# jurihock/sdft

Measured on AMD Instinct MI355X. Metric: Msamples/s analysis+synthesis, m=1024 Hann fp64; achieved HBM GB/s vs peak, higher is better.
Workload: dtype f64

## Files before the change

### sdft_amd/csrc/sdft_forward.hpp

```cpp

#pragma once

#include "sdft_carry_exact.hpp"

#pragma clang fp contract(off)

namespace sdfthip {

template <typename FD, int WIN> SDFT_D cx<FD> window_tap(cx<FD> m2, cx<FD> m1, cx<FD> c0, cx<FD> p1, cx<FD> p2, FD w)
{
  if constexpr (WIN == WIN_HANN)
  {
    const cx<FD> a = cadd(c0, c0);
    const cx<FD> b = cadd(m1, p1);
    return cscale(csub(a, b), w);
  }
  else if constexpr (WIN == WIN_HAMMING)
  {
    const cx<FD> a = cscale(c0, (FD)(0.54));
    const cx<FD> b = cscale(cadd(m1, p1), (FD)(0.23));
    return cscale(csub(a, b), w);
  }
  else if constexpr (WIN == WIN_BLACKMAN)
  {
    const cx<FD> a = cscale(c0, (FD)(0.42));
    const cx<FD> b = cscale(cadd(m1, p1), (FD)(0.25));
    const cx<FD> d = cscale(cadd(m2, p2), (FD)(0.04));
    return cscale(cadd(csub(a, b), d), w);
  }
  else
  {
    return cscale(c0, w);
  }
}

template <typename FD, int WIN> SDFT_D cx<FD> window_tap_fused(cx<FD> m2, cx<FD> m1, cx<FD> c0, cx<FD> p1, cx<FD> p2, FD w)
{
  if constexpr (WIN == WIN_HANN)
  {
    const cx<FD> b = cadd(m1, p1);
    const FD w2 = w + w;
    return cmake<FD>(__builtin_fma(c0.re, w2, -(b.re * w)), __builtin_fma(c0.im, w2, -(b.im * w)));
  }
  else if constexpr (WIN == WIN_HAMMING)
  {
    const cx<FD> b = cadd(m1, p1);
    const FD wa = (FD)(0.54) * w, wb = (FD)(0.23) * w;
    return cmake<FD>(__builtin_fma(c0.re, wa, -(b.re * wb)), __builtin_fma(c0.im, wa, -(b.im * wb)));
  }
  else if constexpr (WIN == WIN_BLACKMAN)
  {
    const cx<FD> b = cadd(m1, p1);
    const cx<FD> d = cadd(m2, p2);
    const FD wa = (FD)(0.42) * w, wb = (FD)(0.25) * w, wd = (FD)(0.04) * w;
    return cmake<FD>(__builtin_fma(d.re, wd, __builtin_fma(c0.re, wa, -(b.re * wb))),
                     __builtin_fma(d.im, wd, __builtin_fma(c0.im, wa, -(b.im * wb))));
  }
  else
  {
    return cscale(c0, w);
  }
}

template <typename FD> SDFT_D cx<FD> fid_from_table(const cx<FD>* fseed, unsigned L, unsigned nbins, long kk, unsigned c, cx<FD> tw)
{
  cx<FD> f = fseed[(size_t)(c / L) * nbins + kk];
  for (unsigned i = c % L; i > 0; --i) f = cmul(f, tw);
  return f;
}

template <typename FD> struct ForwardArgs
{
  const FD* delta;
  const cx<FD>* tw;
  const cx<FD>* wtab;
  const cx<FD>* carry;
  const cx<FD>* seed;
  const cx<FD>* fseed;
  unsigned fseed_L;
  cx<FD>* out;
  size_t out_stride;
  cx<FD>* const* out_rows;
  cx<FD>* acc_state;
  cx<FD>* fid_state;
  size_t n;
  unsigned long long total_waves;
  unsigned nbins, chunks, chunk_len, tiles, interior_lanes, cursor0;
  unsigned chunk0, launch_chunks;
  unsigned chunk_shift;
  int vec_store;
  FD wscale;
  DoneSignal done;
  const unsigned* ready;
  unsigned ready_seq, ready_n, ready_channels;
  unsigned* ready_status;
  unsigned ready_status_seen;
  unsigned xcd_map;
  unsigned inv_chunks, inv_channels;
};
SDFT_D unsigned xcd_contiguous(unsigned b, unsigned total)
{
  const unsigned q = total >> 3, r = total & 7u, x = b & 7u;
  return x * q + (x < r ? x : r) + (b >> 3);
}

SDFT_D void uniform_divmod(unsigned block, unsigned d, unsigned inv, unsigned& q, unsigned& r)
{
  if (inv == 0) { q = block; r = 0; return; }
  q = __builtin_amdgcn_readfirstlane((unsigned)(((unsigned long long)block * inv) >> 32));
  r = block - q * d;
  if (r >= d) { --q; r += d; }
}
template <typename FD> SDFT_D void flow_position(const ForwardArgs<FD>& a, unsigned& chunk, size_t& ch, unsigned block)
{
  unsigned q, r;
  if (a.ready) { uniform_divmod(block, a.ready_channels, a.inv_channels, q, r); chunk = a.chunk0 + q; ch = r; }
  else
  {
    if (a.xcd_map) block = xcd_contiguous(block, a.xcd_map);
    uniform_divmod(block, a.launch_chunks, a.inv_chunks, q, r);
    chunk = a.chunk0 + r; ch = q;
  }
}
template <typename FD> SDFT_D void flow_position(const ForwardArgs<FD>& a, unsigned& chunk, size_t& ch) { flow_position(a, chunk, ch, blockIdx.x); }
constexpr unsigned kFlowPollCap = 1u << 19;
template <typename FD> SDFT_D bool flow_wait(const ForwardArgs<FD>& a, unsigned chunk, size_t ch)
{
  if (!a.ready) return true;
  const unsigned* row = a.ready + (ch * a.chunks + chunk) * (size_t)a.ready_n;
  for (unsigned polls = 0;; ++polls)
  {
    bool ok = true;
    for (unsigned i = threadIdx.x; i < a.ready_n; i += blockDim.x)
      ok = ok && __hip_atomic_load(row + i, __ATOMIC_RELAXED, __HIP_MEMORY_SCOPE_AGENT) == a.ready_seq;
    if (__syncthreads_and(ok ? 1 : 0)) break;
    if (polls > kFlowPollCap)
    {
      if (threadIdx.x == 0 && a.ready_status) __hip_atomic_fetch_add(a.ready_status, 1u, __ATOMIC_RELAXED, __HIP_MEMORY_SCOPE_SYSTEM);
      return false;
    }
    if ((polls & 1023u) == 1023u && a.ready_status)
    {
      const bool gone = threadIdx.x == 0 && __hip_atomic_load(a.ready_status, __ATOMIC_RELAXED, __HIP_MEMORY_SCOPE_SYSTEM) != a.ready_status_seen;
      if (__syncthreads_or(gone ? 1 : 0)) return false;
    }
    __builtin_amdgcn_s_sleep(32);
  }
  __builtin_amdgcn_fence(__ATOMIC_ACQUIRE, "agent");
  asm volatile("s_waitcnt vmcnt(0)" ::: "memory");
  __syncthreads();
  return true;
}

template <typename TD, typename FD> struct SelfArgs
{
  const TD* x;
  size_t x_stride;
  const TD* hist_in;
  TD* hist_out;
  const cx<FD>* acc_in;
  unsigned log2m;
  unsigned lds_deltas;
  const FD* prefix;
#ifdef SDFT_SELF_STAMPS
  unsigned long long* stamps;
#endif
  RadixList rl;
};

template <int CP, int QB, typename TD, typename FD>
SDFT_D void self_fold(const SelfArgs<TD, FD>& sa, cx<FD>* cells, unsigned m, unsigned cursor0, size_t ch, size_t t0)
{
  const TD* xs = sa.x + ch * sa.x_stride;
  const TD* hs = sa.hist_in + ch * (size_t)m;
  const unsigned nthr = blockDim.x;
  const size_t rows = (t0 + m - 1) / m;
  for (unsigned v0 = threadIdx.x; v0 < m; v0 += CP * nthr)
  {
    size_t tv[CP]; FD sum[CP]; TD prev[CP];
#pragma unroll
    for (int c = 0; c < CP; ++c)
    {
      const unsigned v = v0 + (unsigned)c * nthr;
      tv[c] = (size_t)(((v < m ? v : v0) + m - cursor0) % m);
      sum[c] = (FD)0;
      prev[c] = hs[tv[c]];
    }
    for (size_t q = 0; q < rows; q += QB)
    {
      TD cur[CP][QB];
#pragma unroll
      for (int c = 0; c < CP; ++c)
#pragma unroll
        for (int qq = 0; qq < QB; ++qq)
        {
          const size_t t = tv[c] + (q + qq) * (size_t)m;
          cur[c][qq] = xs[t < t0 ? t : t0 - 1];
        }
#pragma unroll
      for (int c = 0; c < CP; ++c)
#pragma unroll
        for (int qq = 0; qq < QB; ++qq)
        {
          const size_t t = tv[c] + (q + qq) * (size_t)m;
          if (t < t0) { const TD dd = cur[c][qq] - prev[c]; sum[c] += (FD)dd; prev[c] = cur[c][qq]; }
        }
    }
#pragma unroll
    for (int c = 0; c < CP; ++c)
    {
      const unsigned v = v0 + (unsigned)c * nthr;
      if (v < m) cells[v] = cmake<FD>(sum[c], (FD)0);
    }
  }
}

template <typename FD>
SDFT_D void lds_fft_dif(cx<FD>* x, unsigned log2m, const cx<FD>* __restrict__ w)
{
  const unsigned m = 1u << log2m;
  unsigned st = 0;
  for (; st + 2 <= log2m; st += 2)
  {
    const unsigned half = m >> (st + 1), quarter = half >> 1;
    for (unsigned i = threadIdx.x; i < (m >> 2); i += blockDim.x)
    {
      const unsigned pos = i & (quarter - 1);
      const unsigned base = ((i - pos) << 2) + pos;
      const cx<FD> a0 = x[base], a1 = x[base + quarter], a2 = x[base + half], a3 = x[base + half + quarter];
      const cx<FD> w1 = w[(size_t)pos << st];
      const cx<FD> w2 = w[(size_t)pos << (st + 1)];
      const cx<FD> b0 = cadd(a0, a2), b2 = cmul(csub(a0, a2), w1);
      const cx<FD> b1 = cadd(a1, a3), tq = cmul(csub(a1, a3), w1);
      const cx<FD> b3 = cmake<FD>(tq.im, -tq.re);
      x[base] = cadd(b0, b1);
      x[base + quarter] = cmul(csub(b0, b1), w2);
      x[base + half] = cadd(b2, b3);
      x[base + half + quarter] = cmul(csub(b2, b3), w2);
    }
    __syncthreads();
  }
  if (st < log2m)
  {
    for (unsigned i = threadIdx.x; i < (m >> 1); i += blockDim.x)
    {
      const cx<FD> p = x[2 * i], q = x[2 * i + 1];
      x[2 * i] = cadd(p, q);
      x[2 * i + 1] = csub(p, q);
    }
    __syncthreads();
  }
}

template <typename FD>
SDFT_D cx<FD>* lds_fft_mixed(cx<FD>* x, unsigned m, const RadixList& rl, const cx<FD>* __restrict__ w)
{
  cx<FD>* y = x + m;
  unsigned ns = 1;
  for (unsigned st = 0; st < rl.count; ++st)
  {
    const unsigned r = rl.r[st];
    const unsigned nr = m / r;
    const unsigned tstep = m / (ns * r);
    const unsigned rstep = nr;
    for (unsigned i = threadIdx.x; i < nr; i += blockDim.x)
    {
      const unsigned k = i % ns;
      cx<FD> v[5];
#pragma unroll
      for (unsigned t = 0; t < 5; ++t)
        if (t < r)
        {
          const cx<FD> in = x[i + t * nr];
          v[t] = t == 0 ? in : cmul(in, w[(size_t)(((unsigned long long)t * k * tstep) % m)]);
        }
      const unsigned base = (i / ns) * ns * r + k;
#pragma unroll
      for (unsigned q = 0; q < 5; ++q)
        if (q < r)
        {
          cx<FD> o = v[0];
#pragma unroll
          for (unsigned t = 1; t < 5; ++t)
            if (t < r) o = cadd(o, cmul(v[t], w[(size_t)(((unsigned long long)q * t * rstep) % m)]));
          y[base + q * ns] = o;
        }
    }
    __syncthreads();
    cx<FD>* tmp = x; x = y; y = tmp;
    ns *= r;
  }
  return x;
}

template <typename TD, typename FD> SDFT_D unsigned self_slot(const SelfArgs<TD, FD>& sa, unsigned k)
{
  return sa.log2m ? (__brev(k) >> (32u - sa.log2m)) : k;
}
template <int CP, int QB, typename TD, typename FD>
SDFT_D cx<FD>* self_carry(const SelfArgs<TD, FD>& sa, const ForwardArgs<FD>& a, cx<FD>* cells, unsigned chunk, size_t ch, size_t t0)
{
  const unsigned m = 2u * a.nbins;
  if (chunk + 1 == a.chunks && sa.hist_out)
  {
    const TD* xv = sa.x + ch * sa.x_stride;
    const TD* hv = sa.hist_in + ch * (size_t)m;
    TD* ho = sa.hist_out + ch * (size_t)m;
    for (size_t i = threadIdx.x; i < m; i += blockDim.x)
    {
      const size_t q = a.n + i;
      ho[i] = (q >= m) ? xv[q - m] : hv[q];
    }
  }
  if (t0 == 0) return nullptr;
#ifdef SDFT_SELF_STAMPS
  const bool st_on = sa.stamps && chunk + 1 == a.chunks && threadIdx.x == 0;
  if (st_on) sa.stamps[1] = __builtin_readcyclecounter();
#endif
  if (sa.prefix)
  {
    const FD* pc = sa.prefix + (ch * a.chunks + chunk) * (size_t)m;
    for (unsigned v = threadIdx.x; v < m; v += blockDim.x) cells[v] = cmake<FD>(pc[v], (FD)0);
  }
  else self_fold<CP, QB>(sa, cells, m, a.cursor0, ch, t0);
  __syncthreads();
#ifdef SDFT_SELF_STAMPS
  if (st_on) sa.stamps[2] = __builtin_readcyclecounter();
#endif
  if (sa.log2m)
  {
    lds_fft_dif(cells, sa.log2m, a.wtab);
#ifdef SDFT_SELF_STAMPS
    if (st_on) sa.stamps[3] = __builtin_readcyclecounter();
#endif
    return cells;
  }
  return lds_fft_mixed(cells, m, sa.rl, a.wtab);
}

template <int G, typename TD, typename FD>
SDFT_D void self_deltas(FD (&dl)[G], const SDFT_CONSTANT TD* xs, const SDFT_CONSTANT TD* hs, size_t tt, size_t span)
{
  TD cur[G], old[G];
#pragma unroll
  for (int u = 0; u < G; ++u) cur[u] = xs[tt + u];
  if (tt + G <= span)
  {
#pragma unroll
    for (int u = 0; u < G; ++u) old[u] = hs[tt + u];
  }
  else if (tt >= span)
  {
#pragma unroll
    for (int u = 0; u < G; ++u) old[u] = xs[tt - span + u];
  }
  else
  {
#pragma unroll
    for (int u = 0; u < G; ++u) old[u] = (tt + u < span) ? hs[tt + u] : xs[tt + u - span];
  }
#pragma unroll
  for (int u = 0; u < G; ++u) { const TD dd = cur[u] - old[u]; dl[u] = (FD)dd; }
}
template <typename TD, typename FD>
SDFT_D FD self_delta1(const SDFT_CONSTANT TD* xs, const SDFT_CONSTANT TD* hs, size_t tt, size_t span)
{
  const TD cur = xs[tt];
  const TD old = (tt < span) ? hs[tt] : xs[tt - span];
  const TD dd = cur - old;
  return (FD)dd;
}

typedef double sdft_v2f64 __attribute__((ext_vector_type(2)));
typedef float sdft_v4f32 __attribute__((ext_vector_type(4)));
typedef float sdft_v2f32 __attribute__((ext_vector_type(2)));
template <typename FD, int BPL> struct StoreVec;
template <> struct StoreVec<double, 1> { using type = sdft_v2f64; };
template <> struct StoreVec<float, 2>  { using type = sdft_v4f32; };
template <> struct StoreVec<float, 1>  { using type = sdft_v2f32; };

template <typename V> SDFT_D void store_vec(V* p, V v) { *p = v; }

template <typename FD, int BPL, int WIN, bool ROWS>
__global__ __launch_bounds__(kBlock) void forward_kernel(ForwardArgs<FD> a)
{
  constexpr int H = win_halo<WIN>::value;
  constexpr int HL = (H + BPL - 1) / BPL;

  const int lane = threadIdx.x & (kWave - 1);
  const unsigned wib = __builtin_amdgcn_readfirstlane(threadIdx.x >> 6);
  const unsigned long long wave = (unsigned long long)blockIdx.x * kWavesPerBlock + wib;
  if (wave >= a.total_waves) return;

  const unsigned tile = (unsigned)(wave % a.tiles);
  const unsigned long long rest = wave / a.tiles;
  const unsigned chunk = a.chunk0 + (unsigned)(rest % a.launch_chunks);
  const size_t ch = (size_t)(rest / a.launch_chunks);

  const long nbins = (long)a.nbins;
  const unsigned span = 2u * a.nbins, maxc = span - 1u;
  const size_t t0 = chunk ? (size_t)chunk * a.chunk_len - a.chunk_shift : 0;
  const size_t tn = (size_t)(chunk + 1) * a.chunk_len - a.chunk_shift;
  const size_t t1 = tn < a.n ? tn : a.n;
  unsigned c = (unsigned)(((size_t)a.cursor0 + t0) % span);

  const long kfirst = (long)tile * a.interior_lanes * BPL + (long)(lane - HL) * BPL;
  const bool owner = (lane >= HL) && (lane < HL + (int)a.interior_lanes);

  BinState<FD> s[BPL];
  bool flip[BPL], live[BPL], keep[BPL];
  const size_t cbase = (ch * a.chunks + chunk) * a.nbins;
#pragma unroll
  for (int b = 0; b < BPL; ++b)
  {
    const long k = kfirst + b;
    const long kk = reflect_bin(k, nbins, flip[b]);
    live[b] = !(nbins == 1 && k != 0);
    keep[b] = owner && k >= 0 && k < nbins;
    s[b].tw = a.tw[kk];
    s[b].acc = a.carry[cbase + kk];
    s[b].fid = a.fseed ? fid_from_table(a.fseed, a.fseed_L, a.nbins, kk, c, s[b].tw)
             : a.seed  ? a.seed[cbase + kk] : a.wtab[(size_t)(((unsigned long long)kk * c) % span)];
  }

  const SDFT_CONSTANT FD* d = as_uniform(a.delta + ch * a.n);
  const FD w = a.wscale;
  const bool last_chunk = (chunk + 1 == a.chunks);

  cx<FD>* dst = a.out + ch * a.out_stride + t0 * (size_t)a.nbins + kfirst;
  cx<FD>* const* rows = ROWS ? a.out_rows + ch * a.n : nullptr;

  auto emit = [&](cx<FD> (&x)[BPL], size_t t)
  {
#pragma unroll
    for (int b = 0; b < BPL; ++b)
    {
      if (flip[b]) x[b].im = -x[b].im;
      if (!live[b]) x[b] = cmake<FD>((FD)0, (FD)0);
    }
    cx<FD> e[BPL + 4] = {};
#pragma unroll
    for (int b = 0; b < BPL; ++b) e[b + 2] = x[b];
    if constexpr (H >= 1)
    {
      e[1] = from_below(x[BPL - 1]);
      e[BPL + 2] = from_above(x[0]);
    }
    if constexpr (H >= 2)
    {
      if constexpr (BPL >= 2)
      {
        e[0] = from_below(x[BPL - 2]);
        e[BPL + 3] = from_above(x[1]);
      }
      else
      {
        e[0] = from_below(e[1]);
        e[BPL + 3] = from_above(e[BPL + 2]);
      }
    }
    cx<FD> y[BPL];
#pragma unroll
    for (int b = 0; b < BPL; ++b)
      y[b] = window_tap<FD, WIN>(e[b], e[b + 1], e[b + 2], e[b + 3], e[b + 4], w);

    cx<FD>* p = dst;
    if constexpr (ROWS) p = rows[t] + kfirst;
    if constexpr (BPL == 2)
    {
      if (a.vec_store && !ROWS)
      {
        if (keep[0])
        {
          using V = typename StoreVec<FD, 2>::type;
          V v; v.x = y[0].re; v.y = y[0].im; v.z = y[1].re; v.w = y[1].im;
          store_vec(reinterpret_cast<V*>(p), v);
        }
      }
      else
      {
        if (keep[0]) p[0] = y[0];
        if (keep[1]) p[1] = y[1];
      }
    }
// ... 66 lines not shown
```

### sdft_amd/csrc/sdft_forward_rows.hpp

```cpp

#pragma once

#include "sdft_ops.hpp"

#pragma clang fp contract(off)

namespace sdfthip {

constexpr int kRowWavesMax = 16;
#ifndef SDFT_ROW_GROUP
#define SDFT_ROW_GROUP 8
#endif
#ifndef SDFT_SYN_GROUP_S2F
#define SDFT_SYN_GROUP_S2F 2
#endif
constexpr int kRowGroup = SDFT_ROW_GROUP;

constexpr int kRowSlotsMax = 2;
#ifndef SDFT_SYN_GROUP_S2D
#define SDFT_SYN_GROUP_S2D 4
#endif
#ifndef SDFT_SYN_GROUP_TREE
#define SDFT_SYN_GROUP_TREE 8
#endif
constexpr int syn_group(int S, int BPL, int SYN)
{
  return (S == 2 && BPL == 2 && SYN == 1) ? SDFT_SYN_GROUP_S2F : (SYN == 1 && S == 1) ? SDFT_SYN_GROUP_TREE
       : (S == 2 && BPL == 1) ? SDFT_SYN_GROUP_S2D : kRowGroup / S;
}

template <typename FD, int BPL, int WIN, bool FUSED, int S, int SYN = 0, bool LAT1 = true, typename TD = float, bool SELF = false>
__global__ __launch_bounds__(kWave * kRowWavesMax) void forward_rows_kernel(ForwardArgs<FD> a, FuseArgs<TD, FD> fz, SelfArgs<TD, FD> sa)
{
  static_assert(!SELF || SYN == 0, "the self-carried form shares the dynamic LDS with the terms image");
  constexpr int H = win_halo<WIN>::value;
  constexpr int G = SYN != 0 ? syn_group(S, BPL, SYN) : ((kRowGroup / (S * BPL)) >= 2 ? kRowGroup / (S * BPL) : 2);
  constexpr int HS = 2;
  constexpr int VW = kRowWavesMax * S;
  __shared__ cx<FD> edgeL[2][G][VW][HS];
  __shared__ cx<FD> edgeR[2][G][VW][HS];
  extern __shared__ __align__(16) unsigned char rows_dyn_lds[];
  FD* terms = reinterpret_cast<FD*>(rows_dyn_lds);

  const int lane = threadIdx.x & (kWave - 1);
  const int wave = __builtin_amdgcn_readfirstlane(threadIdx.x >> 6);
  const int nwaves = blockDim.x >> 6;
  const int nv = nwaves * S;
  unsigned chunk; size_t ch;
  flow_position(a, chunk, ch);
#ifdef SDFT_SELF_STAMPS
  if constexpr (SELF) { if (sa.stamps && chunk + 1 == a.chunks && threadIdx.x == 0) sa.stamps[0] = __builtin_readcyclecounter(); }
#endif
  if (!flow_wait(a, chunk, ch)) return;

  const long nbins = (long)a.nbins;
  const unsigned span = 2u * a.nbins, maxc = span - 1u;
  const size_t t0 = chunk ? (size_t)chunk * a.chunk_len - a.chunk_shift : 0;
  const size_t tn = (size_t)(chunk + 1) * a.chunk_len - a.chunk_shift;
  const size_t t1 = tn < a.n ? tn : a.n;
  unsigned c = (unsigned)(((size_t)a.cursor0 + t0) % span);

  cx<FD>* cells = reinterpret_cast<cx<FD>*>(rows_dyn_lds);
  cx<FD>* dft = nullptr;
  if constexpr (SELF) dft = self_carry<2, (sizeof(TD) == 8 ? 8 : 16)>(sa, a, cells, chunk, ch, t0);

  const long vlast_bin = (long)nv * kWave * BPL - 1;
  BinState<FD> s[S][BPL];
  bool keep[S][BPL], flip[S][BPL];
  cx<FD>* pub[S][BPL];
  bool pubflip[S][BPL], has_role[S][BPL];
  unsigned flipmask[S][BPL], pubmask[S][BPL];
  const size_t cbase = (ch * a.chunks + chunk) * a.nbins;
#pragma unroll
  for (int q = 0; q < S; ++q)
  {
    const int v = q * nwaves + wave;
    const long wfirst = (long)v * kWave * BPL;
    const long wlast = wfirst + (long)kWave * BPL - 1;
#pragma unroll
    for (int b = 0; b < BPL; ++b)
    {
      const long k = wfirst + (long)lane * BPL + b;
      const long kk = reflect_bin(k, nbins, flip[q][b]);
      keep[q][b] = k < nbins;
      s[q][b].tw = a.tw[kk];
      if constexpr (SELF)
      {
        s[q][b].acc = sa.acc_in[ch * a.nbins + kk];
        if (dft) s[q][b].acc = cadd(s[q][b].acc, dft[self_slot(sa, (unsigned)kk)]);
        s[q][b].fid = a.wtab[((unsigned)kk * c) % span];
      }
      else
      {
      s[q][b].acc = a.carry[cbase + kk];
      s[q][b].fid = a.fseed ? fid_from_table(a.fseed, a.fseed_L, a.nbins, kk, c, s[q][b].tw)
                  : a.seed  ? a.seed[cbase + kk] : a.wtab[((unsigned)kk * c) % span];
      }

      pub[q][b] = &edgeL[0][0][0][0];
      pubflip[q][b] = false; has_role[q][b] = false;
      if (H >= 1)
      {
#pragma unroll
        for (int i = 0; i < HS; ++i)
        {
          if (v + 1 < nv && k == wlast - i) { pub[q][b] = &edgeL[0][0][v + 1][i]; has_role[q][b] = true; }
          if (v > 0 && k == wfirst + i) { pub[q][b] = &edgeR[0][0][v - 1][i]; has_role[q][b] = true; }
        }
#pragma unroll
        for (int i = 0; i < HS; ++i)
        {
          bool f0; const long r0 = reflect_bin(-1 - i, nbins, f0);
          if (k == r0) { pub[q][b] = &edgeL[0][0][0][i]; pubflip[q][b] = f0; has_role[q][b] = true; }
          if (vlast_bin - (nbins - 1) < H)
          {
            bool f1; const long r1 = reflect_bin(vlast_bin + 1 + i, nbins, f1);
            if (k == r1) { pub[q][b] = &edgeR[0][0][nv - 1][i]; pubflip[q][b] = f1; has_role[q][b] = true; }
          }
        }
      }
    }
  }
#pragma unroll
  for (int q = 0; q < S; ++q)
#pragma unroll
    for (int b = 0; b < BPL; ++b)
    {
      flipmask[q][b] = flip[q][b] ? 0x80000000u : 0u;
      pubmask[q][b] = (flip[q][b] != pubflip[q][b]) ? 0x80000000u : 0u;
    }
  constexpr size_t kSlabU = (size_t)VW * HS;
  constexpr size_t kSlabBuf = (size_t)G * kSlabU;

  const SDFT_CONSTANT FD* d = as_uniform(a.delta + ch * a.n);
  const SDFT_CONSTANT TD* xin = SELF ? as_uniform(sa.x + ch * sa.x_stride) : nullptr;
  const SDFT_CONSTANT TD* hin = SELF ? as_uniform(sa.hist_in + ch * (size_t)span) : nullptr;
  const FD w = a.wscale;
  cx<FD>* row = a.out + ch * a.out_stride + t0 * (size_t)a.nbins;
  unsigned off_elems[S];
#pragma unroll
  for (int q = 0; q < S; ++q)
  {
    off_elems[q] = (unsigned)(((q * nwaves + wave) * kWave + lane) * BPL);
    __builtin_assume(off_elems[q] < (1u << 20));
  }

  const unsigned term_bins = (unsigned)(nv * kWave * BPL);
  const unsigned term_stride = term_bins + 16u / (unsigned)sizeof(FD);
  GainCursor<FD> gcur;
  const int opk = op_kind_of(fz.op);
  const bool op_has_rows = opk == OP_GAIN || opk == OP_CGAIN;
  gcur.g = nullptr; gcur.left = 0;
  if constexpr (SYN != 0) { if (op_has_rows) gcur.start(fz.op, t0, a.nbins); }
  size_t gtime = t0;

  auto publish = [&](const cx<FD> (&x)[S][BPL], int buf, int u)
  {
    if constexpr (H >= 1)
    {
#pragma unroll
      for (int q = 0; q < S; ++q)
#pragma unroll
        for (int b = 0; b < BPL; ++b)
        {
          if (has_role[q][b])
          {
            cx<FD> v = x[q][b];
            v.im = flip_sign(v.im, pubmask[q][b]);
            pub[q][b][(size_t)buf * kSlabBuf + (size_t)u * kSlabU] = v;
          }
        }
    }
  };

  auto finish = [&](auto optag, const cx<FD> (&xin)[S][BPL], int buf, int u)
  {
    constexpr int kOp = decltype(optag)::value;
    const int opk = kOp >= 0 ? kOp : op_kind_of(fz.op);
    const bool op_has_rows = opk == OP_GAIN || opk == OP_CGAIN;
    if constexpr (SYN != 0) { if (op_has_rows) gcur.seek(gtime); ++gtime; }
#pragma unroll
    for (int q = 0; q < S; ++q)
    {
      const int v = q * nwaves + wave;
      cx<FD> x[BPL];
#pragma unroll
      for (int b = 0; b < BPL; ++b) { x[b] = xin[q][b]; x[b].im = flip_sign(x[b].im, flipmask[q][b]); }
      cx<FD> e[BPL + 4] = {};
#pragma unroll
      for (int b = 0; b < BPL; ++b) e[b + 2] = x[b];
      if constexpr (H >= 1)
      {
        const cx<FD> l0 = edgeL[buf][u][v][0], r0 = edgeR[buf][u][v][0];
        if constexpr (BPL == 1)
        {
          e[1] = from_below_fill(l0, x[0]);
          e[3] = from_above_fill(r0, x[0]);
          if constexpr (H >= 2)
          {
            const cx<FD> l1 = edgeL[buf][u][v][1], r1 = edgeR[buf][u][v][1];
            e[0] = from_below_fill(l1, e[1]);
            e[4] = from_above_fill(r1, e[3]);
          }
        }
        else
        {
          e[1] = from_below_fill(l0, x[BPL - 1]);
          e[BPL + 2] = from_above_fill(r0, x[0]);
          if constexpr (H >= 2)
          {
            const cx<FD> l1 = edgeL[buf][u][v][1], r1 = edgeR[buf][u][v][1];
            e[0] = from_below_fill(l1, x[BPL - 2]);
            e[BPL + 3] = from_above_fill(r1, x[1]);
          }
        }
      }
      cx<FD> y[BPL];
#pragma unroll
      for (int b = 0; b < BPL; ++b)
      {
        if constexpr (FUSED) y[b] = window_tap_fused<FD, WIN>(e[b], e[b + 1], e[b + 2], e[b + 3], e[b + 4], w);
        else y[b] = window_tap<FD, WIN>(e[b], e[b + 1], e[b + 2], e[b + 3], e[b + 4], w);
      }
      if constexpr (SYN != 0)
      {
#pragma unroll
        for (int b = 0; b < BPL; ++b)
        {
          const unsigned k = off_elems[q] + (unsigned)b;
          if (opk == OP_GAIN) y[b] = cscale(y[b], gcur.g[keep[q][b] ? k : 0]);
          else if (opk == OP_CGAIN) y[b] = cmul(y[b], reinterpret_cast<const cx<FD>*>(gcur.g)[keep[q][b] ? k : 0]);
#ifdef SDFT_USER_EXPR
          else if (opk == OP_USER) y[b] = user_op(y[b], k < a.nbins ? k : 0u, a.nbins, gtime - 1, ch, fz.op);
#endif
          else if (opk >= OP_GATE) y[b] = op_pointwise(y[b], fz.op, opk);
          SpectralOp<FD> shift_only = fz.op; shift_only.kind = op_kind_of(fz.op) == OP_SHIFT ? OP_SHIFT : OP_IDENTITY;
          shift_only.gain = nullptr;
          const FD term = synth_term<FD, LAT1, true>(y[b], k, shift_only, fz.syn, a.nbins);
          terms[((size_t)buf * G + (size_t)u) * term_stride + k] = keep[q][b] ? term : (FD)0;
        }
      }
      if (SYN == 0 || fz.store)
      {
      cx<FD>* p = row + off_elems[q];
      if constexpr (BPL == 2)
      {
// ... 71 lines not shown
      {
        if (wave == 0 && lane < gm)
        {
          typedef FD tvec __attribute__((ext_vector_type(16 / sizeof(FD))));
          constexpr int NV = 16 / (int)sizeof(FD);
          const FD* tr = tbase + (size_t)lane * term_stride;
          FD sum = (FD)0;
          for (unsigned k0 = 0; k0 < term_bins; k0 += 8 * NV)
          {
            tvec tv[8];
#pragma unroll
            for (int i = 0; i < 8; ++i) tv[i] = *reinterpret_cast<const tvec*>(tr + k0 + i * NV);
#pragma unroll
            for (int i = 0; i < 8; ++i)
#pragma unroll
              for (int e = 0; e < NV; ++e) sum += tv[i][e];
          }
          yo[lane] = (TD)(sum * fz.sweight);
        }
      }
      else
      {
        for (int u = wave; u < gm; u += nwaves)
        {
          const FD* tr = tbase + (size_t)u * term_stride;
          FD part = (FD)0;
          for (unsigned k = lane; k < term_bins; k += kWave) part += tr[k];
          const FD sum = wave_sum_f(part);
          if (lane == 0) yo[u] = (TD)(sum * fz.sweight);
        }
      }
    }
  };
  bool have_prev = false;
  int prev_m = 0;
  size_t prev_t = 0;

  int buf = 0;
  size_t t = t0;
#ifdef SDFT_SELF_STAMPS
  if constexpr (SELF) { if (sa.stamps && chunk + 1 == a.chunks && threadIdx.x == 0) sa.stamps[4] = __builtin_readcyclecounter(); }
#endif
  while (t < t1)
  {
#ifdef SDFT_SELF_STAMPS
    if constexpr (SELF) { if (sa.stamps && chunk + 1 == a.chunks && threadIdx.x == 0 && t == t0 + (size_t)G) sa.stamps[5] = __builtin_readcyclecounter(); }
#endif
    const int m = (t1 - t < (size_t)G) ? (int)(t1 - t) : G;
    cx<FD> xs[G][S][BPL];
    if (m == G && c + G <= maxc)
    {
      FD dl[G];
      if constexpr (SELF) self_deltas<G>(dl, xin, hin, t, (size_t)span);
      else
      {
#pragma unroll
        for (int u = 0; u < G; ++u) dl[u] = d[t + u];
      }
#pragma unroll
      for (int u = 0; u < G; ++u)
      {
#pragma unroll
        for (int q = 0; q < S; ++q)
#pragma unroll
          for (int b = 0; b < BPL; ++b) xs[u][q][b] = advance(s[q][b], dl[u], false);
        publish(xs[u], buf, u);
      }
      c += G;
    }
    else
    {
#pragma unroll
      for (int u = 0; u < G; ++u)
      {
        if (u < m)
        {
          const FD dl = SELF ? self_delta1<TD, FD>(xin, hin, t + u, (size_t)span) : d[t + u];
          const bool wrap = (c == maxc);
#pragma unroll
          for (int q = 0; q < S; ++q)
#pragma unroll
            for (int b = 0; b < BPL; ++b) xs[u][q][b] = advance(s[q][b], dl, wrap);
          c = wrap ? 0 : c + 1;
          publish(xs[u], buf, u);
        }
      }
    }
    __syncthreads();
    auto phase_b = [&](auto optag)
    {
      if (m == G)
      {
#pragma unroll
        for (int u = 0; u < G; ++u) finish(optag, xs[u], buf, u);
      }
      else
      {
#pragma unroll
        for (int u = 0; u < G; ++u)
          if (u < m) finish(optag, xs[u], buf, u);
      }
    };
    if constexpr (SYN != 0 && SDFT_FIXED_OP < 0)
    {
      switch (opk)
      {
        case OP_GAIN:  phase_b(OpTag<OP_GAIN>{}); break;
        case OP_CGAIN: phase_b(OpTag<OP_CGAIN>{}); break;
        case OP_GATE:  phase_b(OpTag<OP_GATE>{}); break;
        case OP_POWER: phase_b(OpTag<OP_POWER>{}); break;
        default:       phase_b(OpTag<OP_IDENTITY>{}); break;
      }
    }
    else phase_b(OpTag<(SYN != 0 && SDFT_FIXED_OP >= 0) ? SDFT_FIXED_OP : OP_IDENTITY>{});
    if constexpr (SYN != 0)
    {
      if (have_prev) sum_group(buf ^ 1, prev_m, prev_t);
      have_prev = true; prev_m = m; prev_t = t;
    }
    t += m;
    buf ^= 1;
  }
  if constexpr (SYN != 0)
  {
    if (have_prev) { __syncthreads(); sum_group(buf ^ 1, prev_m, prev_t); }
  }

  if (chunk + 1 == a.chunks && a.acc_state)
  {
#pragma unroll
    for (int q = 0; q < S; ++q)
#pragma unroll
      for (int b = 0; b < BPL; ++b)
        if (keep[q][b])
        {
          const size_t k = (size_t)(q * nwaves + wave) * kWave * BPL + (size_t)lane * BPL + b;
          a.acc_state[ch * a.nbins + k] = s[q][b].acc;
          a.fid_state[ch * a.nbins + k] = s[q][b].fid;
        }
  }
#ifdef SDFT_SELF_STAMPS
  if constexpr (SELF) { if (sa.stamps && chunk + 1 == a.chunks && threadIdx.x == 0) sa.stamps[6] = __builtin_readcyclecounter(); }
#endif
  signal_done_workgroup(a.done);
}

template <typename TD, typename FD>
__global__ __launch_bounds__(kWave * kRowWavesMax) void self_state_kernel(ForwardArgs<FD> a, SelfArgs<TD, FD> sa)
{
  extern __shared__ __align__(16) unsigned char rows_dyn_lds[];
  cx<FD>* cells = reinterpret_cast<cx<FD>*>(rows_dyn_lds);
  const size_t ch = blockIdx.x;
  const unsigned span = 2u * a.nbins;
  const cx<FD>* dft = self_carry<2, (sizeof(TD) == 8 ? 8 : 16)>(sa, a, cells, a.chunks - 1u, ch, a.n);
  const unsigned c = (unsigned)(((size_t)a.cursor0 + a.n) % span);
  for (unsigned k = threadIdx.x; k < a.nbins; k += blockDim.x)
  {
    cx<FD> acc = sa.acc_in[ch * a.nbins + k];
    if (dft) acc = cadd(acc, dft[self_slot(sa, k)]);
    a.acc_state[ch * a.nbins + k] = acc;
    a.fid_state[ch * a.nbins + k] = a.wtab[(size_t)(((unsigned long long)k * c) % span)];
  }
}

template <typename FD> __global__ __launch_bounds__(kWave) void queue_probe_kernel(unsigned long long ticks)
{
  const unsigned long long t0 = wall_clock64();
  while (wall_clock64() - t0 < ticks) __builtin_amdgcn_s_sleep(32);
}

}
```

### sdft_amd/csrc/sdft_fused.hpp

```cpp

#pragma once

#include "sdft_forward_rows.hpp"

#pragma clang fp contract(off)

namespace sdfthip {

template <int CTRL> SDFT_D float dpp_move(float v) { return __int_as_float(__builtin_amdgcn_update_dpp(0, __float_as_int(v), CTRL, 0xf, 0xf, true)); }
template <int CTRL> SDFT_D double dpp_move(double v)
{
  const int lo = __builtin_amdgcn_update_dpp(0, __double2loint(v), CTRL, 0xf, 0xf, true);
  const int hi = __builtin_amdgcn_update_dpp(0, __double2hiint(v), CTRL, 0xf, 0xf, true);
  return __hiloint2double(hi, lo);
}
template <typename FD> SDFT_D FD sum_of_eight(FD v)
{
  v += dpp_move<0xB1>(v);
  v += dpp_move<0x4E>(v);
  v += dpp_move<0x141>(v);
  return v;
}

template <typename TD, typename FD> struct ProcArgs
{
  TD* y;
  size_t y_stride;
  const double* alpha;
  const double* beta;
  FD sweight;
  unsigned rows;
  size_t hop;
};

template <typename FD>
__global__ __launch_bounds__(kBlock) void fold_coeff_kernel(double* alpha, double* beta, SpectralOp<FD> op, const cx<FD>* syn,
                                                            unsigned nbins, int lat1, FD h0, FD h1, FD h2)
{
  const long r = (long)blockIdx.x * kBlock + threadIdx.x, N = (long)nbins;
  if (r >= N) return;
  if (op.rows > 1 && op.gain) op.gain += (size_t)blockIdx.y * (size_t)nbins * (op.kind == OP_CGAIN ? 2u : 1u);
  alpha += (size_t)blockIdx.y * nbins; beta += (size_t)blockIdx.y * nbins;
  const double h[5] = {(double)h2, (double)h1, (double)h0, (double)h1, (double)h2};
  double al = 0.0, be = 0.0;
  auto add_position = [&](long m, bool flip)
  {
    for (int i = -2; i <= 2; ++i)
    {
      const long j = m - i;
      if (j < 0 || j >= N) continue;
      const long ko = j + (op.kind == OP_SHIFT ? op.shift : 0);
      if (ko < 0 || ko >= N) continue;
      double A, B;
      if (lat1) { A = (ko & 1) ? -1.0 : +1.0; B = 0.0; }
      else { A = (double)syn[ko].re; B = -(double)syn[ko].im; }
      if (op.kind == OP_GAIN) { A *= (double)op.gain[j]; B *= (double)op.gain[j]; }
      else if (op.kind == OP_CGAIN)
      {
        const cx<FD> g = reinterpret_cast<const cx<FD>*>(op.gain)[j];
        const double cr = (double)g.re * A + (double)g.im * B, ci = (double)g.im * A - (double)g.re * B;
        A = cr; B = -ci;
      }
      al += h[i + 2] * A;
      be += (flip ? -(h[i + 2] * B) : h[i + 2] * B);
    }
  };
  add_position(r, false);
  if (r >= 1 && r <= 2) add_position(-r, true);
  const long mr = 2 * (N - 1) - r;
  if (mr >= N && mr <= N + 1) add_position(mr, true);
  alpha[r] = al;
  beta[r] = be;
}

#ifndef SDFT_PROC_RING
#define SDFT_PROC_RING 4
#endif
constexpr int kProcGroup = 8;
constexpr int kProcRow = 72;
constexpr int kProcRing = SDFT_PROC_RING;
constexpr int kProcSync = SDFT_PROC_RING / 2;

template <typename TD, typename FD, int J, bool FUSED, bool HASB, bool SELF = false>
__global__ __launch_bounds__(kWave * kRowWavesMax, J == 1 ? 8 : 4) void process_rows_kernel(ForwardArgs<FD> a, ProcArgs<TD, FD> pz, SelfArgs<TD, FD> sa)
{
  constexpr int G = kProcGroup;
  constexpr int R = kProcRing, K = kProcSync;
  using AT = double;
  extern __shared__ __align__(16) unsigned char proc_dyn_lds[];
  AT* const tiles = reinterpret_cast<AT*>(proc_dyn_lds);
  __shared__ AT part[R][kRowWavesMax][G];

  const int lane = threadIdx.x & (kWave - 1);
  const int wave = __builtin_amdgcn_readfirstlane(threadIdx.x >> 6);
  const int nwaves = blockDim.x >> 6;
  unsigned chunk; size_t ch;
  flow_position(a, chunk, ch);
  if (!flow_wait(a, chunk, ch)) return;

  const unsigned span = 2u * a.nbins, maxc = span - 1u;
  const size_t t0 = chunk ? (size_t)chunk * a.chunk_len - a.chunk_shift : 0;
  const size_t tn = (size_t)(chunk + 1) * a.chunk_len - a.chunk_shift;
  const size_t t1 = tn < a.n ? tn : a.n;
  unsigned c = (unsigned)(((size_t)a.cursor0 + t0) % span);

  for (int i = threadIdx.x; i < R * G * kRowWavesMax; i += blockDim.x) (&part[0][0][0])[i] = (AT)0;
  FD* const dl_lds = reinterpret_cast<FD*>(tiles + (size_t)(blockDim.x >> 6) * G * kProcRow);
  const bool staged = SELF && sa.lds_deltas != 0 && (t1 - t0) <= (size_t)sa.lds_deltas;
  if constexpr (SELF)
  {
    if (staged)
    {
      const TD* xs = sa.x + ch * sa.x_stride;
      const TD* hs = sa.hist_in + ch * (size_t)span;
      for (size_t i = threadIdx.x; i < t1 - t0; i += blockDim.x)
      {
        const size_t tt = t0 + i;
        const TD dd = xs[tt] - (tt < span ? hs[tt] : xs[tt - span]);
        dl_lds[i] = (FD)dd;
      }
    }
  }

  cx<FD>* cells = reinterpret_cast<cx<FD>*>(tiles);
  cx<FD>* dft = nullptr;
  if constexpr (SELF) dft = self_carry<1, 8>(sa, a, cells, chunk, ch, t0);

  BinState<FD> s[J];
  AT al[J], be[J];
  bool live[J];
  const size_t cbase = (ch * a.chunks + chunk) * a.nbins;
#pragma unroll
  for (int j = 0; j < J; ++j)
  {
    const unsigned k = (unsigned)((j * nwaves + wave) * kWave + lane);
    live[j] = k < a.nbins;
    const unsigned kk = live[j] ? k : 0u;
    s[j].tw = a.tw[kk];
    if constexpr (SELF)
    {
      s[j].acc = sa.acc_in[ch * a.nbins + kk];
      if (dft) s[j].acc = cadd(s[j].acc, dft[self_slot(sa, kk)]);
      s[j].fid = a.wtab[(size_t)(((unsigned long long)kk * c) % span)];
    }
    else
    {
    s[j].acc = a.carry[cbase + kk];
    s[j].fid = a.fseed ? fid_from_table(a.fseed, a.fseed_L, a.nbins, (long)kk, c, s[j].tw)
             : a.seed  ? a.seed[cbase + kk] : a.wtab[(size_t)(((unsigned long long)kk * c) % span)];
    }
    if (!live[j]) { s[j].tw = cmake<FD>((FD)0, (FD)0); s[j].acc = s[j].tw; s[j].fid = s[j].tw; }
    if constexpr (FUSED)
    {
      s[j].acc = cmake<FD>(__builtin_fma(s[j].acc.re, s[j].fid.re, s[j].acc.im * s[j].fid.im),
                           __builtin_fma(s[j].acc.im, s[j].fid.re, -(s[j].acc.re * s[j].fid.im)));
      s[j].tw.im = -s[j].tw.im;
    }
  }
  size_t coeff_row = 0, coeff_next = ~(size_t)0;
  if (pz.rows > 1)
  {
    coeff_row = t0 / pz.hop;
    if (coeff_row >= pz.rows) coeff_row = pz.rows - 1;
    if (coeff_row + 1 < pz.rows) coeff_next = (coeff_row + 1) * pz.hop;
  }
  auto load_coeff = [&]()
  {
#pragma unroll
    for (int j = 0; j < J; ++j)
    {
      const unsigned k = (unsigned)((j * nwaves + wave) * kWave + lane);
      al[j] = live[j] ? pz.alpha[coeff_row * a.nbins + k] : (AT)0;
      be[j] = live[j] ? pz.beta[coeff_row * a.nbins + k] : (AT)0;
    }
  };
  load_coeff();
  __syncthreads();

  auto step_all = [&](FD dl, bool wrap) -> AT
  {
    AT vv = (AT)0;
#pragma unroll
    for (int j = 0; j < J; ++j)
    {
      BinState<FD>& b = s[j];
      if constexpr (FUSED)
      {
        (void)wrap;
        const FD xr0 = b.acc.re + dl;
        const FD nr = __builtin_fma(xr0, b.tw.re, -(b.acc.im * b.tw.im));
        const FD ni = __builtin_fma(xr0, b.tw.im, b.acc.im * b.tw.re);
        b.acc.re = nr; b.acc.im = ni;
        vv = __builtin_fma(al[j], nr, vv);
        if constexpr (HASB) vv = __builtin_fma(be[j], ni, vv);
      }
      else
      {
        if (wrap) advance_wrap(b, dl); else advance_normal(b, dl);
        const AT ar = (AT)b.acc.re, ai = (AT)b.acc.im, fr = (AT)b.fid.re, fi = (AT)b.fid.im;
        const AT xr = ar * fr + ai * fi;
        vv += al[j] * xr;
        if constexpr (HASB)
        {
          const AT xi = ai * fr - ar * fi;
          vv += be[j] * xi;
        }
      }
    }
    return vv;
  };

  const SDFT_CONSTANT FD* d = as_uniform(a.delta + ch * a.n);
  const SDFT_CONSTANT TD* xin = SELF ? as_uniform(sa.x + ch * sa.x_stride) : nullptr;
  const SDFT_CONSTANT TD* hin = SELF ? as_uniform(sa.hist_in + ch * (size_t)span) : nullptr;
  TD* yo = pz.y + ch * pz.y_stride;
  AT* my = tiles + (size_t)wave * G * kProcRow;
  const int ru = lane >> 3, rs = lane & 7;
  auto finish_groups = [&](unsigned first, unsigned count)
  {
    for (unsigned g = first + (unsigned)wave; g < first + count; g += (unsigned)nwaves)
    {
      const size_t tg = t0 + (size_t)g * G;
      const int mg = (t1 - tg < (size_t)G) ? (int)(t1 - tg) : G;
      AT p = part[g % R][rs][ru] + part[g % R][rs + 8][ru];
      p = sum_of_eight(p);
      if (rs == 0 && ru < mg) yo[tg + ru] = (TD)(p * (AT)pz.sweight);
    }
  };
  unsigned gi = 0;
  size_t t = t0;
  while (t < t1)
  {
    const int m = (t1 - t < (size_t)G) ? (int)(t1 - t) : G;
    AT v[G];
    if (m == G && c + G <= maxc && t + G <= coeff_next)
    {
      FD dl[G];
      if constexpr (SELF)
      {
        if (staged)
        {
#pragma unroll
          for (int u = 0; u < G; ++u) dl[u] = dl_lds[t - t0 + u];
        }
        else self_deltas<G>(dl, xin, hin, t, (size_t)span);
      }
      else
      {
#pragma unroll
        for (int u = 0; u < G; ++u) dl[u] = d[t + u];
      }
#pragma unroll
      for (int u = 0; u < G; ++u) v[u] = step_all(dl[u], false);
      c += G;
    }
    else
    {
#pragma unroll
      for (int u = 0; u < G; ++u)
      {
        v[u] = (AT)0;
        if (u < m)
        {
          if (t + u == coeff_next)
          {
            ++coeff_row;
            coeff_next = (coeff_row + 1 < pz.rows) ? coeff_next + pz.hop : ~(size_t)0;
            load_coeff();
          }
          const FD dl = SELF ? self_delta1<TD, FD>(xin, hin, t + u, (size_t)span) : d[t + u];
          const bool wrap = (c == maxc);
          v[u] = step_all(dl, wrap);
          c = wrap ? 0 : c + 1;
        }
      }
    }
#pragma unroll
    for (int u = 0; u < G; ++u) my[u * kProcRow + lane] = v[u];
    AT sum = my[ru * kProcRow + rs * 8 + (rs & 7)];
// ... 218 lines not shown
```

Before: 421.2.

## Prefetch twiddles, history, and bin state to overlap latency in self-carry path

Restructures the self-carry prologue so global loads are issued early and their latency overlaps other work. The fold loop becomes double-buffered with 32-bit indexing and sched barriers, FFT twiddles for the first few radix-4 phases are loaded into registers ahead of time, and history copy-out values are loaded up front. Per-bin tw/acc/fid loads are hoisted before the carry computation, and prefix loads are batched. This raises register pressure and assumes indices fit in 32 bits, which could lower occupancy or overflow on long inputs.

```diff
diff --git a/sdft_amd/csrc/sdft_forward.hpp b/sdft_amd/csrc/sdft_forward.hpp
--- a/sdft_amd/csrc/sdft_forward.hpp
+++ b/sdft_amd/csrc/sdft_forward.hpp
@@ -168,43 +168,85 @@
   RadixList rl;
 };
 
+template <typename T> SDFT_D T load_at(const T* base, unsigned i)
+{
+  return *reinterpret_cast<const T*>(reinterpret_cast<const char*>(base) + (size_t)(i * (unsigned)sizeof(T)));
+}
+
 template <int CP, int QB, typename TD, typename FD>
 SDFT_D void self_fold(const SelfArgs<TD, FD>& sa, cx<FD>* cells, unsigned m, unsigned cursor0, size_t ch, size_t t0)
 {
+  static_assert(QB >= 2 && QB % 2 == 0, "two batches of QB/2 rows");
+  constexpr int HB = QB / 2;
   const TD* xs = sa.x + ch * sa.x_stride;
   const TD* hs = sa.hist_in + ch * (size_t)m;
   const unsigned nthr = blockDim.x;
-  const size_t rows = (t0 + m - 1) / m;
+  const unsigned t0u = (unsigned)t0;
+  const unsigned rows = (t0u + m - 1) / m;
+  const unsigned last = t0u - 1;
   for (unsigned v0 = threadIdx.x; v0 < m; v0 += CP * nthr)
   {
-    size_t tv[CP]; FD sum[CP]; TD prev[CP];
+    unsigned tv[CP]; FD sum[CP]; TD prev[CP];
 #pragma unroll
     for (int c = 0; c < CP; ++c)
     {
       const unsigned v = v0 + (unsigned)c * nthr;
-      tv[c] = (size_t)(((v < m ? v : v0) + m - cursor0) % m);
+      const unsigned f = (v < m ? v : v0) + m - cursor0;
+      tv[c] = f >= m ? f - m : f;
       sum[c] = (FD)0;
-      prev[c] = hs[tv[c]];
-    }
-    for (size_t q = 0; q < rows; q += QB)
-    {
-      TD cur[CP][QB];
+      prev[c] = load_at(hs, tv[c]);
+    }
+    unsigned nxt[CP], cnt[CP];
+#pragma unroll
+    for (int c = 0; c < CP; ++c) { nxt[c] = tv[c]; cnt[c] = tv[c] + (rows - 1) * m < t0u ? rows : rows - 1; }
+    auto fetch = [&](TD (&cur)[CP][HB])
+    {
 #pragma unroll
       for (int c = 0; c < CP; ++c)
-#pragma unroll
-        for (int qq = 0; qq < QB; ++qq)
+      {
+        asm volatile("" : "+v"(nxt[c]));
+#pragma unroll
+        for (int qq = 0; qq < HB; ++qq)
         {
-          const size_t t = tv[c] + (q + qq) * (size_t)m;
-          cur[c][qq] = xs[t < t0 ? t : t0 - 1];
+          const unsigned t = nxt[c] + (unsigned)qq * m;
+          cur[c][qq] = load_at(xs, t < last ? t : last);
         }
-#pragma unroll
-      for (int c = 0; c < CP; ++c)
-#pragma unroll
-        for (int qq = 0; qq < QB; ++qq)
-        {
-          const size_t t = tv[c] + (q + qq) * (size_t)m;
-          if (t < t0) { const TD dd = cur[c][qq] - prev[c]; sum[c] += (FD)dd; prev[c] = cur[c][qq]; }
-        }
+        nxt[c] += (unsigned)HB * m;
+      }
+    };
+    auto add = [&](const TD (&cur)[CP][HB], unsigned q)
+    {
+      asm volatile("" : "+s"(q));
+      if (q + HB < rows)
+      {
+#pragma unroll
+        for (int c = 0; c < CP; ++c)
+#pragma unroll
+          for (int qq = 0; qq < HB; ++qq) { const TD dd = cur[c][qq] - prev[c]; sum[c] += (FD)dd; prev[c] = cur[c][qq]; }
+      }
+      else
+      {
+#pragma unroll
+        for (int c = 0; c < CP; ++c)
+#pragma unroll
+          for (int qq = 0; qq < HB; ++qq)
+            if (q + qq < cnt[c]) { const TD dd = cur[c][qq] - prev[c]; sum[c] += (FD)dd; prev[c] = cur[c][qq]; }
+      }
+    };
+    TD ca[CP][HB], cb[CP][HB];
+    fetch(ca);
+    fetch(cb);
+    for (unsigned q = 0; q < rows; q += 2 * HB)
+    {
+      __builtin_amdgcn_sched_barrier(0);
+      add(ca, q);
+      __builtin_amdgcn_sched_barrier(0);
+      fetch(ca);
+      if (q + HB >= rows) break;
+      __builtin_amdgcn_sched_barrier(0);
+      add(cb, q + HB);
+      __builtin_amdgcn_sched_barrier(0);
+      fetch(cb);
     }
 #pragma unroll
     for (int c = 0; c < CP; ++c)
@@ -215,31 +257,86 @@
   }
 }
 
-template <typename FD>
-SDFT_D void lds_fft_dif(cx<FD>* x, unsigned log2m, const cx<FD>* __restrict__ w)
+#ifndef SDFT_SELF_PHASES
+#define SDFT_SELF_PHASES 6
+#endif
+#ifndef SDFT_SELF_PHASES_D
+#define SDFT_SELF_PHASES_D 5
+#endif
+#ifndef SDFT_SELF_PHASES_S2
+#define SDFT_SELF_PHASES_S2 4
+#endif
+#ifndef SDFT_SELF_PHASES_FUSED
+#define SDFT_SELF_PHASES_FUSED 3
+#endif
+#ifndef SDFT_SELF_PHASES_FUSED_D
+#define SDFT_SELF_PHASES_FUSED_D 1
+#endif
+#ifndef SDFT_SELF_PHASES_FUSED2
+#define SDFT_SELF_PHASES_FUSED2 3
+#endif
+#ifndef SDFT_SELF_PHASES_FUSED2_D
+#define SDFT_SELF_PHASES_FUSED2_D 3
+#endif
+constexpr int self_phases_rows(int slots, int td_bytes) { return slots != 1 ? SDFT_SELF_PHASES_S2 : td_bytes == 8 ? SDFT_SELF_PHASES_D : SDFT_SELF_PHASES; }
+constexpr int self_phases_fused(int bins, int td_bytes)
+{
+  return bins == 1 ? (td_bytes == 8 ? SDFT_SELF_PHASES_FUSED_D : SDFT_SELF_PHASES_FUSED) : (td_bytes == 8 ? SDFT_SELF_PHASES_FUSED2_D : SDFT_SELF_PHASES_FUSED2);
+}
+template <typename FD, int NPH> struct SelfTwiddles { cx<FD> w1[NPH > 0 ? NPH : 1], w2[NPH > 0 ? NPH : 1]; };
+template <int NPH, typename FD>
+SDFT_D void lds_fft_dif_request(SelfTwiddles<FD, NPH>& tw, unsigned log2m, const cx<FD>* __restrict__ w)
+{
+  const unsigned m = log2m ? 1u << log2m : 0u;
+#pragma unroll
+  for (int p = 0; p < NPH; ++p)
+  {
+    const unsigned st = 2u * (unsigned)p;
+    const bool has = st + 2 <= log2m && threadIdx.x < (m >> 2);
+    const unsigned quarter = has ? m >> (st + 2) : 1u;
+    const unsigned pos = threadIdx.x & (quarter - 1);
+    tw.w1[p] = load_at(w, pos << st);
+    tw.w2[p] = load_at(w, pos << (st + 1));
+  }
+}
+
+template <int NPH, typename FD>
+SDFT_D void lds_fft_dif(cx<FD>* x, unsigned log2m, const cx<FD>* __restrict__ w, const SelfTwiddles<FD, NPH>& tw)
 {
   const unsigned m = 1u << log2m;
+  auto butterfly = [&](unsigned base, unsigned half, unsigned quarter, cx<FD> w1, cx<FD> w2)
+  {
+    const cx<FD> a0 = x[base], a1 = x[base + quarter], a2 = x[base + half], a3 = x[base + half + quarter];
+    const cx<FD> b0 = cadd(a0, a2), b2 = cmul(csub(a0, a2), w1);
+    const cx<FD> b1 = cadd(a1, a3), tq = cmul(csub(a1, a3), w1);
+    const cx<FD> b3 = cmake<FD>(tq.im, -tq.re);
+    x[base] = cadd(b0, b1);
+    x[base + quarter] = cmul(csub(b0, b1), w2);
+    x[base + half] = cadd(b2, b3);
+    x[base + half + quarter] = cmul(csub(b2, b3), w2);
+  };
+  auto phase = [&](unsigned st, bool pre, cx<FD> p1, cx<FD> p2)
+  {
+    const unsigned half = m >> (st + 1), quarter = half >> 1;
+    unsigned i = threadIdx.x;
+    if (pre && i < (m >> 2))
+    {
+      const unsigned pos = i & (quarter - 1);
+      butterfly(((i - pos) << 2) + pos, half, quarter, p1, p2);
+      i += blockDim.x;
+    }
+    for (; i < (m >> 2); i += blockDim.x)
+    {
+      const unsigned pos = i & (quarter - 1);
+      butterfly(((i - pos) << 2) + pos, half, quarter, w[(size_t)pos << st], w[(size_t)pos << (st + 1)]);
+    }
+    __syncthreads();
+  };
   unsigned st = 0;
-  for (; st + 2 <= log2m; st += 2)
-  {
-    const unsigned half = m >> (st + 1), quarter = half >> 1;
-    for (unsigned i = threadIdx.x; i < (m >> 2); i += blockDim.x)
-    {
-      const unsigned pos = i & (quarter - 1);
-      const unsigned base = ((i - pos) << 2) + pos;
-      const cx<FD> a0 = x[base], a1 = x[base + quarter], a2 = x[base + half], a3 = x[base + half + quarter];
-      const cx<FD> w1 = w[(size_t)pos << st];
-      const cx<FD> w2 = w[(size_t)pos << (st + 1)];
-      const cx<FD> b0 = cadd(a0, a2), b2 = cmul(csub(a0, a2), w1);
-      const cx<FD> b1 = cadd(a1, a3), tq = cmul(csub(a1, a3), w1);
-      const cx<FD> b3 = cmake<FD>(tq.im, -tq.re);
-      x[base] = cadd(b0, b1);
-      x[base + quarter] = cmul(csub(b0, b1), w2);
-      x[base + half] = cadd(b2, b3);
-      x[base + half + quarter] = cmul(csub(b2, b3), w2);
-    }
-    __syncthreads();
-  }
+#pragma unroll
+  for (int p = 0; p < NPH; ++p)
+    if (st + 2 <= log2m) { phase(st, true, tw.w1[p], tw.w2[p]); st += 2; }
+  for (; st + 2 <= log2m; st += 2) phase(st, false, cx<FD>{}, cx<FD>{});
   if (st < log2m)
   {
     for (unsigned i = threadIdx.x; i < (m >> 1); i += blockDim.x)
@@ -297,22 +394,47 @@
 {
   return sa.log2m ? (__brev(k) >> (32u - sa.log2m)) : k;
 }
-template <int CP, int QB, typename TD, typename FD>
+template <int CP, int QB, int NPH, int HC = 2, typename TD, typename FD>
 SDFT_D cx<FD>* self_carry(const SelfArgs<TD, FD>& sa, const ForwardArgs<FD>& a, cx<FD>* cells, unsigned chunk, size_t ch, size_t t0)
 {
   const unsigned m = 2u * a.nbins;
-  if (chunk + 1 == a.chunks && sa.hist_out)
+  const unsigned nthr = blockDim.x;
+  SelfTwiddles<FD, NPH> ftw;
+  lds_fft_dif_request<NPH>(ftw, sa.log2m, a.wtab);
+  TD hc[HC > 0 ? HC : 1];
   {
     const TD* xv = sa.x + ch * sa.x_stride;
     const TD* hv = sa.hist_in + ch * (size_t)m;
-    TD* ho = sa.hist_out + ch * (size_t)m;
-    for (size_t i = threadIdx.x; i < m; i += blockDim.x)
-    {
-      const size_t q = a.n + i;
-      ho[i] = (q >= m) ? xv[q - m] : hv[q];
-    }
-  }
-  if (t0 == 0) return nullptr;
+#pragma unroll
+    for (int j = 0; j < HC; ++j)
+    {
+      const unsigned i = threadIdx.x + (unsigned)j * nthr;
+      const size_t q = a.n + (i < m ? i : 0u);
+      const TD* src = (q >= m) ? xv + (q - m) : hv + q;
+      hc[j] = *src;
+    }
+  }
+  auto put_hist = [&]()
+  {
+    if (chunk + 1 == a.chunks && sa.hist_out)
+    {
+      const TD* xv = sa.x + ch * sa.x_stride;
+      const TD* hv = sa.hist_in + ch * (size_t)m;
+      TD* ho = sa.hist_out + ch * (size_t)m;
+#pragma unroll
+      for (int j = 0; j < HC; ++j)
+      {
+        const unsigned i = threadIdx.x + (unsigned)j * nthr;
+        if (i < m) ho[i] = hc[j];
+      }
+      for (size_t i = threadIdx.x + (size_t)HC * nthr; i < m; i += nthr)
+      {
+        const size_t q = a.n + i;
+        ho[i] = (q >= m) ? xv[q - m] : hv[q];
+      }
+    }
+  };
+  if (t0 == 0) { put_hist(); return nullptr; }
 #ifdef SDFT_SELF_STAMPS
   const bool st_on = sa.stamps && chunk + 1 == a.chunks && threadIdx.x == 0;
   if (st_on) sa.stamps[1] = __builtin_readcyclecounter();
@@ -320,16 +442,23 @@
   if (sa.prefix)
   {
     const FD* pc = sa.prefix + (ch * a.chunks + chunk) * (size_t)m;
-    for (unsigned v = threadIdx.x; v < m; v += blockDim.x) cells[v] = cmake<FD>(pc[v], (FD)0);
+    constexpr int PC = 4;
+    FD pv[PC];
+#pragma unroll
+    for (int j = 0; j < PC; ++j) { const unsigned v = threadIdx.x + (unsigned)j * nthr; pv[j] = load_at(pc, v < m ? v : 0u); }
+#pragma unroll
+    for (int j = 0; j < PC; ++j) { const unsigned v = threadIdx.x + (unsigned)j * nthr; if (v < m) cells[v] = cmake<FD>(pv[j], (FD)0); }
+    for (unsigned v = threadIdx.x + (unsigned)PC * nthr; v < m; v += nthr) cells[v] = cmake<FD>(pc[v], (FD)0);
   }
   else self_fold<CP, QB>(sa, cells, m, a.cursor0, ch, t0);
+  put_hist();
   __syncthreads();
 #ifdef SDFT_SELF_STAMPS
   if (st_on) sa.stamps[2] = __builtin_readcyclecounter();
 #endif
   if (sa.log2m)
   {
-    lds_fft_dif(cells, sa.log2m, a.wtab);
+    lds_fft_dif<NPH>(cells, sa.log2m, a.wtab, ftw);
 #ifdef SDFT_SELF_STAMPS
     if (st_on) sa.stamps[3] = __builtin_readcyclecounter();
 #endif
diff --git a/sdft_amd/csrc/sdft_forward_rows.hpp b/sdft_amd/csrc/sdft_forward_rows.hpp
--- a/sdft_amd/csrc/sdft_forward_rows.hpp
+++ b/sdft_amd/csrc/sdft_forward_rows.hpp
@@ -62,7 +62,22 @@
 
   cx<FD>* cells = reinterpret_cast<cx<FD>*>(rows_dyn_lds);
   cx<FD>* dft = nullptr;
-  if constexpr (SELF) dft = self_carry<2, (sizeof(TD) == 8 ? 8 : 16)>(sa, a, cells, chunk, ch, t0);
+  cx<FD> pre_tw[S][BPL], pre_acc[S][BPL], pre_fid[S][BPL];
+  if constexpr (SELF)
+  {
+#pragma unroll
+    for (int q = 0; q < S; ++q)
+#pragma unroll
+      for (int b = 0; b < BPL; ++b)
+      {
+        bool f;
+        const long kk = reflect_bin((long)(q * nwaves + wave) * kWave * BPL + (long)lane * BPL + b, nbins, f);
+        pre_tw[q][b] = load_at(a.tw, (unsigned)kk);
+        pre_acc[q][b] = load_at(sa.acc_in + ch * a.nbins, (unsigned)kk);
+        pre_fid[q][b] = load_at(a.wtab, ((unsigned)kk * c) % span);
+      }
+  }
+  if constexpr (SELF) dft = self_carry<2, (sizeof(TD) == 8 ? 8 : 16), self_phases_rows(S, (int)sizeof(TD))>(sa, a, cells, chunk, ch, t0);
 
   const long vlast_bin = (long)nv * kWave * BPL - 1;
   BinState<FD> s[S][BPL];
@@ -83,15 +98,16 @@
       const long k = wfirst + (long)lane * BPL + b;
       const long kk = reflect_bin(k, nbins, flip[q][b]);
       keep[q][b] = k < nbins;
+      if constexpr (SELF)
+      {
+        s[q][b].tw = pre_tw[q][b];
+        s[q][b].acc = pre_acc[q][b];
+        if (dft) s[q][b].acc = cadd(s[q][b].acc, dft[self_slot(sa, (unsigned)kk)]);
+        s[q][b].fid = pre_fid[q][b];
+      }
+      else
+      {
       s[q][b].tw = a.tw[kk];
-      if constexpr (SELF)
-      {
-        s[q][b].acc = sa.acc_in[ch * a.nbins + kk];
-        if (dft) s[q][b].acc = cadd(s[q][b].acc, dft[self_slot(sa, (unsigned)kk)]);
-        s[q][b].fid = a.wtab[((unsigned)kk * c) % span];
-      }
-      else
-      {
       s[q][b].acc = a.carry[cbase + kk];
       s[q][b].fid = a.fseed ? fid_from_table(a.fseed, a.fseed_L, a.nbins, kk, c, s[q][b].tw)
                   : a.seed  ? a.seed[cbase + kk] : a.wtab[((unsigned)kk * c) % span];
@@ -469,7 +485,7 @@
   cx<FD>* cells = reinterpret_cast<cx<FD>*>(rows_dyn_lds);
   const size_t ch = blockIdx.x;
   const unsigned span = 2u * a.nbins;
-  const cx<FD>* dft = self_carry<2, (sizeof(TD) == 8 ? 8 : 16)>(sa, a, cells, a.chunks - 1u, ch, a.n);
+  const cx<FD>* dft = self_carry<2, (sizeof(TD) == 8 ? 8 : 16), self_phases_rows(1, (int)sizeof(TD))>(sa, a, cells, a.chunks - 1u, ch, a.n);
   const unsigned c = (unsigned)(((size_t)a.cursor0 + a.n) % span);
   for (unsigned k = threadIdx.x; k < a.nbins; k += blockDim.x)
   {
diff --git a/sdft_amd/csrc/sdft_fused.hpp b/sdft_amd/csrc/sdft_fused.hpp
--- a/sdft_amd/csrc/sdft_fused.hpp
+++ b/sdft_amd/csrc/sdft_fused.hpp
@@ -124,7 +124,7 @@
 
   cx<FD>* cells = reinterpret_cast<cx<FD>*>(tiles);
   cx<FD>* dft = nullptr;
-  if constexpr (SELF) dft = self_carry<1, 8>(sa, a, cells, chunk, ch, t0);
+  if constexpr (SELF) dft = self_carry<1, 8, self_phases_fused(J, (int)sizeof(TD)), (J == 1 && sizeof(TD) == 8 ? 0 : 2)>(sa, a, cells, chunk, ch, t0);
 
   BinState<FD> s[J];
   AT al[J], be[J];
```

New measurement: 420.0. Within noise of the previous version (-0.3%).
